# thisparticle/scl_slam

Measured on AMD Instinct MI355X. Metric: loop-closure candidates/sec: (scan, keyframe) pairs taken through full-database ARG-MIN detection per second (every pair aligned exactly and bounded by the f16 matrix-core screening; only the survivors get the f64 distance), batches of 16 scans, 10k-keyframe DB per GPU, higher is better.
Workload: dtype f64 results; f16-operand / f32-accumulate MFMA screening + f64 exact pass on the survivors

## Files before the change

### scl_slam_amd/csrc/engine.hip

```cpp
#include "scl_engine.h"

#include <hip/hip_runtime.h>

#include <cfloat>
#include <climits>
#include <chrono>
#include <cmath>
#include <cstdio>
#include <cstdlib>
#include <cstring>
#include <mutex>
#include <new>
#include <string>
#include <atomic>
#include <chrono>
#include <thread>
#include <vector>

#include "db_file.hpp"
#include "engine_internal.hpp"
#include "device_sort.hpp"
#include "plugin_host.hpp"

#ifdef SCL_DIAGNOSTICS
// ... 383 lines not shown
    return SCL_OK;
}

int topk_finish_locked(scl_engine *e, int k, bool have_dist, int *idx, float *d2, double *dist, int *shift, int *found)
{
    int rc;
    char *h = static_cast<char *>(e->h_pinned);
    bool seen = false;
    if (e->pinned_seq) {
        const volatile unsigned int *w = reinterpret_cast<const volatile unsigned int *>(h + cand_seq_offset(k));
        const auto t0 = std::chrono::steady_clock::now();
        int spins = 0;
        seen = true;
        while (*w != e->pinned_seq)
            if ((++spins & 255) == 0 && std::chrono::steady_clock::now() - t0 > std::chrono::microseconds(300)) { seen = false; break; }
        std::atomic_thread_fence(std::memory_order_acquire);
        if (seen) collect_profile(e);
    }
    if (!seen && (rc = sync_short(e))) return rc;
    const int *h_idx = reinterpret_cast<int *>(h);
    const float *h_d2 = reinterpret_cast<float *>(h + sizeof(int) * k);
    const double *h_dist = reinterpret_cast<double *>(h + (sizeof(int) + sizeof(float)) * k);
    const int *h_shift = reinterpret_cast<int *>(h + (sizeof(int) + sizeof(float) + sizeof(double)) * k);
    int nf = 0;
    for (int i = 0; i < k; ++i) {
        if (idx) idx[i] = h_idx[i];
        if (d2) d2[i] = h_d2[i];
        if (dist) dist[i] = have_dist ? h_dist[i] : kBigDist;
        if (shift) shift[i] = have_dist ? h_shift[i] : 0;
        if (h_idx[i] >= 0) nf++;
    }
    if (found) *found = nf;
    return SCL_OK;
}

int topk_with_distance_locked(scl_engine *e, int query, int lo, int hi, int k, float eps,
                              int *idx, float *d2, double *dist, int *shift, int *found)
{
    bool have_dist = false;
    int rc = topk_enqueue_locked(e, query, lo, hi, k, eps, dist || shift, &have_dist);
    if (rc) return rc;
    return topk_finish_locked(e, k, have_dist, idx, d2, dist, shift, found);
}

}

extern "C" {

const char *scl_status_string(int status)
{
    switch (status) {
    case SCL_OK: return "ok";
    case SCL_ERR_INVALID_ARG: return "invalid argument";
    case SCL_ERR_NO_DEVICE: return "no HIP device";
    case SCL_ERR_HIP: return "HIP runtime error";
    case SCL_ERR_OUT_OF_RANGE: return "index out of range";
    case SCL_ERR_NOMEM: return "out of memory";
    case SCL_ERR_UNSUPPORTED: return "unsupported";
    default: return "unknown status";
    }
}

const char *scl_last_error(const scl_engine *e) { return e ? e->last_error.c_str() : "null engine"; }

int scl_abi_version(void) { return 12; }

int scl_default_config(scl_config *c)
{
    if (!c) return SCL_ERR_INVALID_ARG;
    c->num_ring = 20; c->num_sector = 60; c->num_candidates = 3;
    c->dist_thres = 0.14; c->lidar_height = 1.65; c->max_radius = 80.0;
    c->num_exclude_recent = 100; c->tree_making_period = 10;
    c->search_ratio = 0.1;
    c->knn_exclude_eps = 0.0f;
    c->device = 0;
    c->initial_capacity = 4096;
    return SCL_OK;
}

static void log_env_overrides_once()
{
    static std::atomic<bool> done{false};
    if (done.exchange(true)) return;
    static const char *const names[] = {"SCL_SCREEN", "SCL_SCREEN_FORM", "SCL_SCREEN_V2_MIN", "SCL_SCREEN_PAIR", "SCL_RCCL_LIB",
                                        "SCL_SCREEN_VARIANT", "SCL_SCREEN_PROBE", "SCL_SCREEN_TAIL", "SCL_ALIGN_WGS",
                                        "SCL_ALIGN2_WGS", "SCL_ALIGN_FILTER", "SCL_SC_KERNEL", "SCL_SC_WAVES", "SCL_STAMP", "SCL_ABLATE",
                                        "SCL_ICP_REDUCE", "SCL_MATRIX_PLAIN", "SCL_MATRIX_KERNEL", "SCL_MATRIX_KR", "SCL_WIDE_EXACT", "SCL_STREAM_EXACT", "SCL_SMALL_EXACT_OFF",
                                        "SCL_SELF_ALIGN_OFF", "SCL_CAND_EXACT_OFF"};
    constexpr int kProduct = 5;
    int i = 0;
    for (const char *n : names) {
        const char *v = getenv(n);
#ifdef SCL_DIAGNOSTICS
        if (v) fprintf(stderr, "scl_engine (diagnostics build): environment override in effect: %s=%s\n", n, v);
#else
        if (v && i < kProduct) fprintf(stderr, "scl_engine: environment override in effect: %s=%s\n", n, v);
        else if (v) fprintf(stderr, "scl_engine: %s=%s is an experiment's switch: ignored by this build (make EXTRA=-DSCL_DIAGNOSTICS builds them in)\n", n, v);
#endif
        ++i;
    }
    (void)kProduct;
}

int scl_create(const scl_config *cfg, scl_engine **out)
{
    if (!cfg || !out) return SCL_ERR_INVALID_ARG;
    *out = nullptr;
    log_env_overrides_once();
    if (cfg->num_ring < 1 || cfg->num_ring > 256 || cfg->num_sector < 1 || cfg->num_sector > 1024 ||
        cfg->num_candidates < 1 || cfg->num_candidates > kTopkMaxK || cfg->tree_making_period < 1 ||
        cfg->num_exclude_recent < 0 || !(cfg->max_radius > 0.0) || !(cfg->search_ratio >= 0.0))
        return SCL_ERR_INVALID_ARG;
    int ndev = 0;
    if (hipGetDeviceCount(&ndev) != hipSuccess || ndev <= 0) return SCL_ERR_NO_DEVICE;
    if (cfg->device < 0 || cfg->device >= ndev) return SCL_ERR_INVALID_ARG;
    scl_engine *e = new (std::nothrow) scl_engine();
    if (!e) return SCL_ERR_NOMEM;
    e->cfg = *cfg;
    e->R = cfg->num_ring; e->S = cfg->num_sector;
    e->RG = (e->R + 3) / 4; e->R4 = e->RG * 4;
    e->hstride = hdesc_stride(e->RG, e->S);
    e->hkw = hkey_row_halfs(e->S);
    e->SR = (int)std::round(0.5 * cfg->search_ratio * (double)e->S);
    if (e->SR < 0) e->SR = 0;
    e->device = cfg->device;
    int rc = SCL_OK;
    auto bail = [&](int code) { scl_destroy(e); return code; };
    if (hipSetDevice(e->device) != hipSuccess) return bail(SCL_ERR_HIP);
    hipDeviceProp_t prop;
    if (hipGetDeviceProperties(&prop, e->device) == hipSuccess && prop.multiProcessorCount > 0)
        e->num_cu = prop.multiProcessorCount;
    if (hipStreamCreateWithFlags(&e->stream, hipStreamNonBlocking) != hipSuccess) return bail(SCL_ERR_HIP);
    {
        int lo_p = 0, hi_p = 0;
        (void)hipDeviceGetStreamPriorityRange(&lo_p, &hi_p);
        if (hipStreamCreateWithPriority(&e->stream2, hipStreamNonBlocking, hi_p) != hipSuccess) return bail(SCL_ERR_HIP);
    }
    if (hipEventCreateWithFlags(&e->ev_fork, hipEventDisableTiming) != hipSuccess) return bail(SCL_ERR_HIP);
    if (hipEventCreateWithFlags(&e->ev_join, hipEventDisableTiming) != hipSuccess) return bail(SCL_ERR_HIP);
    if (hipHostMalloc((void **)&e->h_out3, 64 * scl_engine::kSlots, hipHostMallocDefault) != hipSuccess) return bail(SCL_ERR_HIP);
    memset(e->h_out3, 0, 64 * scl_engine::kSlots);
    for (int i = 0; i < scl_engine::kSlots; ++i)
        if (hipEventCreateWithFlags(&e->ev_done[i], hipEventDisableTiming) != hipSuccess) return bail(SCL_ERR_HIP);
    if ((rc = ensure_capacity(e, 1))) return bail(rc);
    if ((rc = dev_alloc(e, &e->d_topk_scratch, (size_t)kTopkMaxBlocks * kTopkMaxK + 2))) return bail(rc);
    if (hipMemset(e->d_topk_scratch, 0, sizeof(unsigned long long) * ((size_t)kTopkMaxBlocks * kTopkMaxK + 2)) != hipSuccess) return bail(SCL_ERR_HIP);
    if ((rc = dev_alloc(e, &e->d_topk_idx, (size_t)kTopkMaxK * scl_engine::kScreenSets))) return bail(rc);
    if ((rc = dev_alloc(e, &e->d_topk_d2, (size_t)kTopkMaxK * scl_engine::kScreenSets))) return bail(rc);
    if ((rc = dev_alloc(e, &e->d_out3, (size_t)4))) return bail(rc);
    if ((rc = dev_alloc(e, &e->d_blk_part, (size_t)kTailBlocks * kTailRec * kMaxQueryBatch))) return bail(rc);
    static_assert(kMaxQueryBatch <= 4, "done_counter holds four counters");
    if ((rc = dev_alloc(e, &e->d_done_counter, (size_t)4))) return bail(rc);
    if (hipMemset(e->d_done_counter, 0, 16) != hipSuccess) return bail(SCL_ERR_HIP);
    {
        constexpr int NS = scl_engine::kScreenSets;
        if ((rc = dev_alloc(e, &e->d_nsurv, (size_t)NS))) return bail(rc);
        static_assert(NS <= kTminEpsOffset, "the launch's largest bound sits kTminEpsOffset words behind its t_min word");
        if ((rc = dev_alloc(e, &e->d_tmin, (size_t)NS + kTminEpsOffset))) return bail(rc);
        if (hipMemset(e->d_nsurv, 0, sizeof(int) * NS) != hipSuccess) return bail(SCL_ERR_HIP);
        if (hipMemset(e->d_tmin, 0xff, sizeof(unsigned int) * NS) != hipSuccess) return bail(SCL_ERR_HIP);
        if (hipMemset(e->d_tmin + NS, 0, sizeof(unsigned int) * kTminEpsOffset) != hipSuccess) return bail(SCL_ERR_HIP);
        if ((rc = dev_alloc(e, &e->d_surv_part, (size_t)NS * kSurvivorBlocks * kTailRec))) return bail(rc);
        if ((rc = dev_alloc(e, &e->d_surv_done, (size_t)NS))) return bail(rc);
        if (hipMemset(e->d_surv_done, 0, sizeof(unsigned int) * NS) != hipSuccess) return bail(SCL_ERR_HIP);
        if (hipMalloc(&e->d_surv_args, (size_t)8 * NS * kSurvivorArgBytes) != hipSuccess) return bail(SCL_ERR_NOMEM);
        if (hipHostMalloc(&e->h_surv_args, (size_t)8 * NS * kSurvivorArgBytes, hipHostMallocDefault) != hipSuccess) return bail(SCL_ERR_HIP);
        if (hipHostMalloc((void **)&e->h_stream_out, (size_t)2 * NS * 64, hipHostMallocDefault) != hipSuccess) return bail(SCL_ERR_HIP);
        for (auto &ev : e->ev_chunk) if (hipEventCreateWithFlags(&ev, hipEventDisableTiming) != hipSuccess) return bail(SCL_ERR_HIP);
        for (auto &ev : e->ev_k1) if (hipEventCreateWithFlags(&ev, hipEventDisableTiming) != hipSuccess) return bail(SCL_ERR_HIP);
        for (auto &ev : e->ev_sub0) if (hipEventCreateWithFlags(&ev, hipEventDisableTiming) != hipSuccess) return bail(SCL_ERR_HIP);
        if (hipEventCreateWithFlags(&e->ev_align_gate, hipEventDisableTiming) != hipSuccess) return bail(SCL_ERR_HIP);
        {
// ... 2470 lines not shown
```

### scl_slam_amd/csrc/sc_screen.hip

```cpp
#include <atomic>
#include <type_traits>

#include "align_exact.hpp"
#include "device_common.hpp"
#include "kernels.hpp"

namespace scl {

namespace {

typedef _Float16 h4 __attribute__((ext_vector_type(4)));
typedef _Float16 h8 __attribute__((ext_vector_type(8)));
typedef float f4v __attribute__((ext_vector_type(4)));
typedef float f2 __attribute__((ext_vector_type(2)));
typedef unsigned int u32x4 __attribute__((ext_vector_type(4)));
typedef u32x4 __attribute__((aligned(8))) u32x4_a8;

struct ScreenArgs {
    const double *vkey;
    const uint2 *hdesc; const unsigned int *kmask;
    const double *q_vkey; const float *q_rkey;
    const uint2 *q_hdesc; const unsigned int *q_kmask;
    const _Float16 *hkey; const _Float16 *q_hkey; int hkw;
    const float4 *rkey4; int rk_cap;
// ... 408 lines not shown
        const float v1 = hi[0], v2 = lo[0] + 7.0e-5f;
        int a1 = (int)(__float_as_uint(hi[0]) & 255u);
        const bool in_range = qnorm >= 1e-30f && qnorm <= 4.0e6f && knorm >= 1e-30f && knorm <= 4.0e6f &&
                              qnorm <= 1.0e4f * knorm && knorm <= 1.0e4f * qnorm;
        const float lead = (qerr > 0.f && kerr > 0.f) ? fminf(kAlign16Margin, 2.0f * (qerr + kerr + qerr * kerr) * 1.0001f + 1.6e-5f) : kAlign16Margin;
        bool uniq = use_filter && in_range && (v1 == v1) && (v2 < v1 - lead);
        const int ci = u_lo + idx - sq.base;
        const bool mine = q_live && ci >= 0 && ci < sq.n;
        unsigned long long amb = __builtin_amdgcn_ballot_w64(mine && !uniq) & 0xffffull;
        if (SCL_A2_PROBE != 1 && use_filter && amb) {
            const uint4 l0 = *reinterpret_cast<const uint4 *>(g_cur + 16 + IMG + loff0);
            uint4 l1 = make_uint4(0, 0, 0, 0);
            if (NLD > 1) l1 = *reinterpret_cast<const uint4 *>(g_cur + 16 + IMG + (ld1 ? loff1 : 0u));
            *reinterpret_cast<uint4 *>(smem_wave + IMG + loff0) = l0;
            if (ld1) *reinterpret_cast<uint4 *>(smem_wave + IMG + loff1) = l1;
            h8 bql[KS];
#pragma unroll
            for (int kk = 0; kk < KS; ++kk) bql[kk] = *reinterpret_cast<const h8 *>(qk + SK + 8 + 32 * kk + 8 * j4);
            wave_fence();
            float h2 = kNegInf, l2 = kNegInf;
            int g2 = 0;
#pragma unroll
            for (int t = 0; t < NT; ++t) {
                const int rho = t / NTAU, tau = t - rho * NTAU;
                const f4v zero = {0.f, 0.f, 0.f, 0.f};
                f4v hh = zero, xx = zero;
#pragma unroll
                for (int kk = 0; kk < KS; ++kk) {
                    const unsigned char *ap = smem_wave + rho * (CP * 2) + offs[kk + C::TSTEP * (NTAU - 1 - tau)];
                    const h8 ah = frag(ap), al = frag(ap + IMG);
                    const f4v one = __builtin_amdgcn_mfma_f32_16x16x32_f16(ah, bq[kk], zero, 0, 0, 0);
                    hh = kk == 0 ? one : hh + one;
                    xx = __builtin_amdgcn_mfma_f32_16x16x32_f16(ah, bql[kk], xx, 0, 0, 0);
                    xx = __builtin_amdgcn_mfma_f32_16x16x32_f16(al, bq[kk], xx, 0, 0, 0);
                }
#pragma unroll
                for (int i = 0; i < 4; ++i) {
                    const int sg = 16 * tau + 4 * j4 + i;
                    const float c = sg < C::ROWS ? __builtin_fmaf(xx[i], 0x1p-11f, hh[i]) : kNegInf;
                    l2 = fmaxf(l2, fminf(c, h2));
                    g2 = c > h2 ? P * sg + rho : g2;
                    h2 = fmaxf(h2, c);
                }
            }
#pragma unroll
            for (int off = 16; off <= 32; off <<= 1) {
                const float oh = __shfl_xor(h2, off, kWave), ol = __shfl_xor(l2, off, kWave);
                const int og = __shfl_xor(g2, off, kWave);
                l2 = fmaxf(fmaxf(l2, ol), fminf(h2, oh));
                g2 = oh > h2 ? og : g2;
                h2 = fmaxf(h2, oh);
            }
            if (!uniq && in_range && (h2 == h2) && (l2 < h2 - 2.0f * kAlignSplitEps)) { uniq = true; a1 = g2; }
            amb = __builtin_amdgcn_ballot_w64(mine && !uniq) & 0xffffull;
        }
        if (mine && j4 == 0 && uniq) starts_q[ci] = wrapS(a1 - SR, S);
        if (SCL_A2_PROBE == 1 && mine && j4 == 0 && !uniq) starts_q[ci] = kAlignUndecided;
        open_pairs += (unsigned long long)__popcll(amb);
        while (SCL_A2_PROBE != 1 && amb) {
            const int qn = __ffsll((long long)amb) - 1;
            amb &= amb - 1;
            const ScreenQuery oq = ab.q[qn];
            const double *vq = ab.vkey + (size_t)oq.slot * S;
            const double *vkp = ab.vkey + (size_t)(u_lo + idx) * S;
            double *vk2 = reinterpret_cast<double *>(smem_wave);
            int al;
            if constexpr (S / 2 <= kWave) {
                constexpr int L = S >> 1;
                const int ll = lane < L ? lane : L - 1;
                const double2 vk = *reinterpret_cast<const double2 *>(vkp + 2 * ll);
                al = align_keyframe_exact<S>(vk, lane, vk2, vq);
            } else {
                constexpr int SPL = (S + kWave - 1) / kWave, LA = S / SPL;
                const int ll = lane < LA ? lane : LA - 1;
                double vk[SPL];
#pragma unroll
                for (int u = 0; u < SPL; ++u) vk[u] = vkp[SPL * ll + u];
                al = align_keyframe_wide<S>(vk, lane, vk2, vq);
            }
            if (lane == 0) (ab.starts + (size_t)oq.buf * (size_t)ab.pair_stride)[u_lo + idx - oq.base] = wrapS(al - SR, S);
        }
    }
    if (lane == 0 && open_pairs && ab.fallbacks) atomicAdd(ab.fallbacks, open_pairs);
}

template <int RG, int S, int W>
__global__ __launch_bounds__(kScreenWaves * kWave, Align2Cfg<S>::OCC) void sc_align2_kernel(ScreenBatchArgs ab, const unsigned char *halign, int u_lo, int u_n)
{
    extern __shared__ __attribute__((aligned(16))) unsigned char smem_align2[];
    const int wave = __builtin_amdgcn_readfirstlane((int)(threadIdx.x >> 6));
    sc_align2_role<S, W>(ab, halign, u_lo, u_n, (int)blockIdx.x * kScreenWaves + wave, (int)gridDim.x * kScreenWaves,
                         smem_align2 + (size_t)wave * Align2Cfg<S>::LDS_WAVE);
}


template <int S>
__device__ __forceinline__ void rotate_mask(const unsigned long long (&m)[(S + 63) / 64], int s, unsigned long long (&out)[(S + 63) / 64])
{
    constexpr int NW = (S + 63) / 64;
    auto shr = [&](int k, unsigned long long (&o)[NW]) {
        const int w = k >> 6, b = k & 63;
#pragma unroll
        for (int i = 0; i < NW; ++i) {
            const unsigned long long lo = i + w < NW ? m[i + w] : 0ull, hi = i + w + 1 < NW ? m[i + w + 1] : 0ull;
            o[i] = b ? (lo >> b) | (hi << (64 - b)) : lo;
        }
    };
    auto shl = [&](int k, unsigned long long (&o)[NW]) {
        const int w = k >> 6, b = k & 63;
#pragma unroll
        for (int i = 0; i < NW; ++i) {
            const unsigned long long hi = i - w >= 0 && i - w < NW ? m[i - w] : 0ull, lo = i - w - 1 >= 0 && i - w - 1 < NW ? m[i - w - 1] : 0ull;
            o[i] = b ? (hi << b) | (lo >> (64 - b)) : hi;
        }
    };
    unsigned long long r1[NW], r2[NW];
    shr(s, r1);
    shl(S - s, r2);
#pragma unroll
    for (int i = 0; i < NW; ++i) {
        unsigned long long v = r1[i] | r2[i];
        const int top = S - 64 * i;
        if (top < 64) v &= top > 0 ? ((1ull << (top & 63)) - 1ull) : 0ull;
        out[i] = v;
    }
}

template <int RGH, int S, int W, int D, int PROBE>
__device__ __forceinline__ void sc_screen_role(const ScreenBatchArgs &ab, const int qi, const int bid, unsigned char *smem_raw)
{
    constexpr int NWV = kScreenWaves;
    constexpr int MT = (W + 15) / 16;
    constexpr int QSX = S + 16 * MT;
    constexpr int SB = RGH * 8;
    constexpr int KH = SB / 64;
    constexpr int QST = SB + 32;
    constexpr int HS = hdesc_stride_rgh(RGH, S);
    constexpr int SPW = S / NWV;
    constexpr int NST = SPW * KH;
    constexpr int NW64 = (S + 63) / 64;
    constexpr int MW = (NW64 + 1) / 2;
    static_assert(S % NWV == 0 && SB % 64 == 0 && NST % D == 0 && W <= 32 && S <= 224, "tiling");

    const int nbk = ab.nb;
    const ScreenArgs a = screen_args_of(ab, qi);
    const int lane = threadIdx.x & (kWave - 1);
    const int wave = __builtin_amdgcn_readfirstlane((int)(threadIdx.x >> 6));

    unsigned char *Qs = smem_raw;
    uint4 *rotq = reinterpret_cast<uint4 *>(Qs + (size_t)QSX * QST);
    unsigned char *tile = reinterpret_cast<unsigned char *>(rotq + S * MW) + (size_t)wave * (kGroup * kTileStride);
    f4v *part = reinterpret_cast<f4v *>(reinterpret_cast<unsigned char *>(rotq + S * MW) + (size_t)NWV * (kGroup * kTileStride));

    for (int idx = threadIdx.x; idx < QSX * (SB / 16); idx += blockDim.x) {
        const int cx = idx / (SB / 16), ch = idx - cx * (SB / 16);
        const int c = cx < S ? cx : cx - S;
        *reinterpret_cast<uint4 *>(Qs + (size_t)cx * QST + ch * 16) =
            *reinterpret_cast<const uint4 *>(reinterpret_cast<const unsigned char *>(a.q_hdesc) + (size_t)c * SB + ch * 16);
    }
    const bool q_bad = a.q_kmask[7] != 0;
    const float q_err = __uint_as_float(a.q_kmask[6]);
    {
        unsigned long long qm[NW64];
#pragma unroll
        for (int i = 0; i < NW64; ++i) qm[i] = (unsigned long long)a.q_kmask[2 * i] | ((unsigned long long)(2 * i + 1 < 7 ? a.q_kmask[2 * i + 1] : 0u) << 32);
        for (int sft = threadIdx.x; sft < S; sft += blockDim.x) {
// ... 833 lines not shown
template <int RG, int S, int W, bool MASKS = true, bool D2 = true>
__device__ __forceinline__ void sc_screen2_finish_body(const Screen2Args &fa, const int qi, const int chunk)
{
    constexpr int NW64 = (S + 63) / 64, MW = (NW64 + 1) / 2;
    const ScreenBatchArgs &ab = fa.prod;
    const ScreenArgs a = screen_args_of(ab, qi);
    __shared__ uint4 rotq[S * MW];
    __shared__ float wmin[4], wmax[4];
    __shared__ float4 qkey[D2 ? RG : 1];
    const int ci = (int)(chunk * blockDim.x + threadIdx.x);
    const bool live = ci < a.n;
    float4 qk_mine = make_float4(0.0f, 0.0f, 0.0f, 0.0f);
    if constexpr (D2) { if (threadIdx.x < RG) qk_mine = reinterpret_cast<const float4 *>(a.q_rkey)[threadIdx.x]; }
    FinishLoads<RG, S, W, D2> ld = sc_screen2_finish_request<RG, S, W, D2>(fa, a, qi, live ? ci : 0);
    build_rotq<S>(a.q_kmask, rotq, (int)threadIdx.x, (int)blockDim.x);
    const bool q_bad = a.q_kmask[7] != 0;
    if constexpr (D2) { if (threadIdx.x < RG) qkey[threadIdx.x] = qk_mine; }
    __syncthreads();
#pragma unroll
    for (int i = 0; i < FinishLoads<RG, S, W, D2>::NPF; ++i) asm("" : "+v"(ld.pv[i]));
    const float kInf = __int_as_float(0x7f800000);
    float contrib = kInf, peps = 0.0f;
    if (live) contrib = sc_screen2_finish_compute<RG, S, W, MASKS, D2>(a, ci, rotq, qkey, q_bad, __uint_as_float(a.q_kmask[6]), ld, peps);
    contrib = -wave_max_f32_dpp(-contrib);
    peps = wave_max_f32_dpp(peps);
    if ((threadIdx.x & 63) == 0) { wmin[threadIdx.x >> 6] = contrib; wmax[threadIdx.x >> 6] = peps; }
    __syncthreads();
    if (threadIdx.x == 0) {
        const float m = fminf(fminf(wmin[0], wmin[1]), fminf(wmin[2], wmin[3]));
        if (m < kInf) atomicMin(a.t_min, float_to_ordered_u(m));
        const float pe = fmaxf(fmaxf(wmax[0], wmax[1]), fmaxf(wmax[2], wmax[3]));
        if (pe > 0.0f) atomicMax(a.t_min + kTminEpsOffset, __float_as_uint(pe));
    }
}

__device__ __forceinline__ bool finish_block_of(const int fb, const int nq, const int chunks, int &qi, int &chunk)
{
    const int x = fb & 7, s = fb >> 3, g = s / nq;
    chunk = 8 * g + x; qi = s - g * nq;
    return chunk < chunks;
}
static int finish_blocks(int chunks, int nq) { return 8 * ((chunks + 7) / 8) * nq; }

template <int RG, int S, int W>
__global__ __launch_bounds__(256) void sc_screen2_finish_kernel(Screen2Args fa, int chunks)
{
    int qi, chunk;
    if (!finish_block_of((int)blockIdx.x, fa.prod.nq, chunks, qi, chunk)) return;
    sc_screen2_finish_body<RG, S, W>(fa, qi, chunk);
}

template <int RG, int S, int W>
__global__ __launch_bounds__(kScreenWaves * kWave, 2) void sc_screen2_tail_kernel(Screen2Args fa, ScreenBatchArgs nb, int align_blocks, int chunks)
{
    extern __shared__ __attribute__((aligned(16))) unsigned char smem_tail[];
    const int b = (int)blockIdx.x;
    if (b < align_blocks) { sc_align_role<RG, S, W>(nb, b, smem_tail); return; }
    int qi, chunk;
    if (!finish_block_of(b - align_blocks, fa.prod.nq, chunks, qi, chunk)) return;
    sc_screen2_finish_body<RG, S, W>(fa, qi, chunk);
}

template <int RG, int S, int W, bool MASKS = true, bool D2 = true>
__global__ __launch_bounds__(kScreenWaves * kWave, Align2Cfg<S>::OCC) void sc_screen2_tail2_kernel(Screen2Args fa, ScreenBatchArgs nb, const unsigned char *halign, int u_lo, int u_n,
                                                                                     int align_blocks, int chunks)
{
    extern __shared__ __attribute__((aligned(16))) unsigned char smem_tail2[];
#ifdef SCL_TAIL_FINISH_FIRST
    const int fblocks = (int)gridDim.x - align_blocks;
    const int b = (int)blockIdx.x < fblocks ? (int)blockIdx.x + align_blocks : (int)blockIdx.x - fblocks;
#else
    const int b = (int)blockIdx.x;
#endif
    if (b < align_blocks) {
        const int wave = __builtin_amdgcn_readfirstlane((int)(threadIdx.x >> 6));
        sc_align2_role<S, W>(nb, halign, u_lo, u_n, b * kScreenWaves + wave, align_blocks * kScreenWaves, smem_tail2 + (size_t)wave * Align2Cfg<S>::LDS_WAVE);
        return;
    }
    int qi, chunk;
    if (!finish_block_of(b - align_blocks, fa.prod.nq, chunks, qi, chunk)) return;
    sc_screen2_finish_body<RG, S, W, MASKS, D2>(fa, qi, chunk);
}

static bool screen_second_form()
{
    static const int form = [] { const char *e = getenv("SCL_SCREEN_FORM"); return e ? atoi(e) : 2; }();
    return form != 1;
}
static bool screen_pair_enabled()
{
    static const int on = [] { const char *e = getenv("SCL_SCREEN_PAIR"); return e ? atoi(e) : 1; }();
    return on != 0;
}
static int screen_v2_min_env()
{
    static const int v = [] { const char *e = getenv("SCL_SCREEN_V2_MIN"); return e ? atoi(e) : 0; }();
    return v;
}
int sc_screen_max_batch(const DbView &db, int SR)
{
    return (sc_screen_is_wide(db, SR) && screen_second_form()) ? S2Cfg<20, 180, 19>::NQ : kMaxScreenBatch;
}
size_t sc_screen_scratch_floats(const DbView &db, int SR)
{
    return sc_screen_is_wide(db, SR) ? (size_t)S2Cfg<20, 180, 19>::NQ * s2_part_floats<20, 180, 19>() : (size_t)S2Cfg<16, 120, 13>::NQ * s2_part_floats<16, 120, 13>();
}

static int fill_screen_args(const DbView &db, const ScreenBatch &sb, int align_filter, ScreenBatchArgs *ab)
{
    ab->vkey = db.vkey; ab->rkey = db.rkey; ab->hdesc = db.hdesc; ab->kmask = db.kmask; ab->rkey4 = db.rkey4; ab->hkey = db.hkey; ab->hkw = hkey_row_halfs(db.S);
    ab->starts = sb.starts; ab->approx = sb.approx; ab->ring_d2 = sb.ring_d2; ab->t_min = sb.t_min; ab->fallbacks = sb.align_fallbacks; ab->smask = sb.smask;
    ab->pair_stride = (unsigned long long)sb.pair_stride;
    ab->S = db.S; ab->R4 = 4 * db.RG; ab->hstride = db.hstride; ab->rk_cap = db.cap; ab->align_filter = align_filter;
    ab->nq = sb.nq;
    int nmax = 0;
    for (int i = 0; i < sb.nq; ++i) {
        if (sb.n[i] <= 0) return -1;
        ab->q[i] = ScreenQuery{sb.slot[i], sb.base[i], sb.n[i], sb.buf[i]};
        nmax = sb.n[i] > nmax ? sb.n[i] : nmax;
    }
    for (int i = sb.nq; i < kMaxScreenBatch; ++i) ab->q[i] = ab->q[0];
    return nmax;
}

struct ScreenPairMate { const ScreenBatch *sb; const ScreenBatch *next; };

template <int RG, int S, int W, int OCC0, int OCC1>
static hipError_t launch_screen_grid(const DbView &db, const ScreenBatch &sb, int align_filter, int num_cu, hipStream_t stream, int phases,
                                     const ScreenBatch *next, const ScreenPairMate *mate = nullptr)
{
    constexpr int RGH = hdesc_rgh(RG);
    ScreenBatchArgs ab{};
    const int nmax = fill_screen_args(db, sb, align_filter, &ab);
    if (nmax < 0) return hipErrorInvalidValue;
    ScreenBatchArgs ab_m{};
    const int nmax_m = mate ? fill_screen_args(db, *mate->sb, align_filter, &ab_m) : 0;
    if (nmax_m < 0) return hipErrorInvalidValue;
    const int ngroups = (nmax + kGroup - 1) / kGroup;
    static_assert(halign_bytes(S) > 0, "alignment image");
    if (db.hstride != hdesc_stride(RG, S) || !sb.starts || !db.halign) return hipErrorInvalidValue;
    static std::atomic<bool> attr_set_dev[64];
    int dev_ = 0; (void)hipGetDevice(&dev_);
    std::atomic<bool> &attr_set = attr_set_dev[dev_ & 63];
    static const int variant = scl_lab_int("SCL_SCREEN_VARIANT", 0);
    void (*kern)(ScreenFusedArgs) = sc_screen_kernel<RG, S, W, 15, OCC0>;
#ifdef SCL_DIAGNOSTICS
    if (variant == 1) kern = sc_screen_kernel<RG, S, W, 15, OCC1>;
    if (variant == 2) kern = sc_screen_kernel<RG, S, W, 5, OCC0>;
    static const int probe = scl_lab_int("SCL_SCREEN_PROBE", 0);
    if (probe == 2) kern = sc_screen_kernel<RG, S, W, 15, OCC0, 2>;
#else
    const int probe = 0;
#endif
    constexpr int MTA = (S + 15) / 16, MT = (W + 15) / 16, QSX = S + 16 * MT, MW = ((S + 63) / 64 + 1) / 2;
    const size_t lds0 = (size_t)S * 8 + (size_t)(32 * MTA) * 4 + (size_t)2 * (16 * MTA + hkey_halfs(S) + 8) * 2 +
                        (size_t)kScreenWaves * ((2 * S + 2) * 8);
    const size_t lds1 = (size_t)QSX * (RGH * 8 + 32) + (size_t)S * MW * 16 + (size_t)kScreenWaves * kGroup * kTileStride +
                        (size_t)(2 * kScreenWaves * MT) * kWave * 16;
    if (!attr_set.load(std::memory_order_acquire)) {
        hipError_t e = hipFuncSetAttribute((const void *)sc_screen_kernel<RG, S, W, 15, OCC0>, hipFuncAttributeMaxDynamicSharedMemorySize, 128 * 1024);
        if (e == hipSuccess) e = hipFuncSetAttribute((const void *)sc_align_kernel<RG, S, W>, hipFuncAttributeMaxDynamicSharedMemorySize, 128 * 1024);
        if (e != hipSuccess) return e;
#ifdef SCL_DIAGNOSTICS
        (void)hipFuncSetAttribute((const void *)sc_screen_kernel<RG, S, W, 15, OCC1>, hipFuncAttributeMaxDynamicSharedMemorySize, 128 * 1024);
        (void)hipFuncSetAttribute((const void *)sc_screen_kernel<RG, S, W, 5, OCC0>, hipFuncAttributeMaxDynamicSharedMemorySize, 128 * 1024);
        (void)hipFuncSetAttribute((const void *)sc_screen_kernel<RG, S, W, 15, OCC0, 2>, hipFuncAttributeMaxDynamicSharedMemorySize, 128 * 1024);
#endif
        attr_set.store(true, std::memory_order_release);
    }
    auto align_blocks = [&](int groups, int nq, bool beside_products) {
        int b = (groups + kScreenWaves - 1) / kScreenWaves;
        static const int cap_env = scl_lab_int("SCL_ALIGN_WGS", 0);
        int cap = cap_env > 0 ? cap_env : (beside_products ? 2 * num_cu / (nq > 0 ? nq : 1) : num_cu);
        if (cap < 1) cap = 1;
        return b > cap ? cap : b;
// ... 36 lines not shown
        hipError_t e = hipGetLastError();
        if (e != hipSuccess) return e;
    }
    if (probe == 4 || !(phases & kScreenProducts)) return hipSuccess;
    if (use_v2) {
        static std::atomic<bool> attr2_dev[64];
        std::atomic<bool> &attr2 = attr2_dev[dev_ & 63];
        if (!attr2.load(std::memory_order_acquire)) {
            hipError_t e = hipFuncSetAttribute((const void *)sc_screen2_kernel<RG, S, W>, hipFuncAttributeMaxDynamicSharedMemorySize, (int)(s2_lds<RG, S, W>()));
            if (e != hipSuccess) return e;
            attr2.store(true, std::memory_order_release);
        }
        Screen2Args f2{}, f2_m{};
        f2.prod = ab; f2.part = sb.part;
        union_of(sb, &f2.u_lo, &f2.u_n);
        const int WGU = 8 * S2Cfg<RG, S, W>::NP * (mate ? 2 : 1);
        int nwg = (num_cu / WGU) * WGU;
        if (nwg < WGU) nwg = WGU;
        f2.nwg = nwg;
        hipError_t e = hipSuccess;
        if constexpr (kPairGrid) {
            if (mate) {
                static std::atomic<bool> attrp_dev[64];
                std::atomic<bool> &attrp = attrp_dev[dev_ & 63];
                if (!attrp.load(std::memory_order_acquire)) {
                    e = hipFuncSetAttribute((const void *)sc_screen2_kernel<RG, S, W, 2>, hipFuncAttributeMaxDynamicSharedMemorySize, (int)(s2_lds<RG, S, W>()));
                    if (e != hipSuccess) return e;
                    attrp.store(true, std::memory_order_release);
                }
                f2_m.prod = ab_m; f2_m.part = mate->sb->part; f2_m.nwg = nwg;
                union_of(*mate->sb, &f2_m.u_lo, &f2_m.u_n);
                Screen2PairArgs fp{};
                fp.prod[0] = ab; fp.prod[1] = ab_m; fp.part[0] = sb.part; fp.part[1] = mate->sb->part; fp.nwg = nwg;
                const int hi0 = f2.u_lo + f2.u_n, hi1 = f2_m.u_lo + f2_m.u_n;
                fp.u_lo = f2.u_lo < f2_m.u_lo ? f2.u_lo : f2_m.u_lo;
                fp.u_n = (hi0 > hi1 ? hi0 : hi1) - fp.u_lo;
                hipLaunchKernelGGL((sc_screen2_kernel<RG, S, W, 2>), dim3(nwg), dim3(S2Cfg<RG, S, W>::WV * kWave), (s2_lds<RG, S, W>()), stream, fp);
            }
        }
        if (!mate) hipLaunchKernelGGL((sc_screen2_kernel<RG, S, W>), dim3(nwg), dim3(S2Cfg<RG, S, W>::WV * kWave), (s2_lds<RG, S, W>()), stream, f2);
        if ((e = hipGetLastError()) != hipSuccess) return e;
        auto launch_tail = [&](const ScreenBatch &sb, const Screen2Args &f2, const int nmax, const ScreenBatch *next) -> hipError_t {
            const bool next_v2 = next && second_form_for(*next);
            const int chunks = (nmax + 255) / 256;
            const dim3 fgrid(finish_blocks(chunks, sb.nq)), ablock(kScreenWaves * kWave);
            if (!next) {
                hipLaunchKernelGGL((sc_screen2_finish_kernel<RG, S, W>), fgrid, dim3(256), 0, stream, f2, chunks);
                return hipGetLastError();
            }
            if (next->nq < 1 || next->nq > kMaxScreenBatch) return hipErrorInvalidValue;
            ScreenBatchArgs nb{};
            const int nmax2 = fill_screen_args(db, *next, align_filter, &nb);
            if (nmax2 < 0) return hipErrorInvalidValue;
            nb.skip_d2 = next_v2 ? 1 : 0;
            int ulo = 0, un = 0, ablocks;
            if (next_v2) {
                union_of(*next, &ulo, &un);
                ablocks = align2_blocks(un);
            } else {
                const int ng2 = (nmax2 + kGroup - 1) / kGroup;
                int per_q = 3 * num_cu / next->nq;
                per_q = per_q < 1 ? 1 : per_q;
                nb.nb = (ng2 + kScreenWaves - 1) / kScreenWaves;
                nb.nb = nb.nb > per_q ? per_q : nb.nb;
                ablocks = nb.nb * next->nq;
            }
            static const int tail_env = scl_lab_int("SCL_SCREEN_TAIL", 1);
            if (tail_env) {
                const dim3 tgrid(ablocks + finish_blocks(chunks, sb.nq));
                const bool d2 = !sb.no_ring_metric;
                if (!next_v2) hipLaunchKernelGGL((sc_screen2_tail_kernel<RG, S, W>), tgrid, ablock, lds0, stream, f2, nb, ablocks, chunks);
                else if (sb.smask && d2) hipLaunchKernelGGL((sc_screen2_tail2_kernel<RG, S, W, true, true>), tgrid, ablock, lds_a2, stream, f2, nb, db.halign, ulo, un, ablocks, chunks);
                else if (sb.smask) hipLaunchKernelGGL((sc_screen2_tail2_kernel<RG, S, W, true, false>), tgrid, ablock, lds_a2, stream, f2, nb, db.halign, ulo, un, ablocks, chunks);
                else if (d2) hipLaunchKernelGGL((sc_screen2_tail2_kernel<RG, S, W, false, true>), tgrid, ablock, lds_a2, stream, f2, nb, db.halign, ulo, un, ablocks, chunks);
                else hipLaunchKernelGGL((sc_screen2_tail2_kernel<RG, S, W, false, false>), tgrid, ablock, lds_a2, stream, f2, nb, db.halign, ulo, un, ablocks, chunks);
                return hipGetLastError();
            }
            hipLaunchKernelGGL((sc_screen2_finish_kernel<RG, S, W>), fgrid, dim3(256), 0, stream, f2, chunks);
            if ((e = hipGetLastError()) != hipSuccess) return e;
            if (next_v2) hipLaunchKernelGGL((sc_align2_kernel<RG, S, W>), dim3(ablocks), ablock, lds_a2, stream, nb, db.halign, ulo, un);
            else hipLaunchKernelGGL((sc_align_kernel<RG, S, W>), dim3(ablocks), ablock, lds0, stream, nb);
            return hipGetLastError();
        };
        if ((e = launch_tail(sb, f2, nmax, next)) != hipSuccess || !mate) return e;
        return launch_tail(*mate->sb, f2_m, nmax_m, mate->next);
    }
    ScreenFusedArgs fa{};
    fa.prod = ab;
    int blocks = num_cu * 2;
    if (blocks > ngroups) blocks = ngroups;
    if (blocks > kScreenMaxBlocks) blocks = kScreenMaxBlocks;
    fa.prod.nb = blocks;
    fa.prod.self_align = self_align ? 1 : 0;
    int extra = 0;
    if (next && probe != 3) {
        if (next->nq < 1 || next->nq > kMaxScreenBatch) return hipErrorInvalidValue;
        const int nmax2 = fill_screen_args(db, *next, align_filter, &fa.next);
        if (nmax2 < 0) return hipErrorInvalidValue;
        fa.next.skip_d2 = next_v2 ? 1 : 0;
        fa.next.nb = align_blocks((nmax2 + kGroup - 1) / kGroup, next->nq, true);
        extra = fa.next.nb * next->nq;
#ifdef SCL_DIAGNOSTICS
        if (probe == 5 || probe == 6) fa.next.align_filter = probe == 5 ? 2 : 3;
#endif
    }
    const size_t lds = (extra || self_align) && lds0 > lds1 ? lds0 : lds1;
    fa.align_blocks = extra;
    const int patterned = fused_patterned_blocks(sb.nq, blocks, extra);
    const int slots = 8 * ((blocks + 7) >> 3);
    const int grid = patterned + (extra > slots ? extra - slots : 0);
    hipLaunchKernelGGL(kern, dim3(grid), dim3(kScreenWaves * kWave), lds, stream, fa);
    return hipGetLastError();
}

hipError_t launch_sc_screen_batch(const DbView &db, const ScreenBatch &sb, int SR, int align_filter, int num_cu, hipStream_t stream, int phases,
                                  const ScreenBatch *next)
{
    if (sb.nq < 1 || sb.nq > kMaxScreenBatch || !sc_screen_supported(db, SR)) return hipErrorInvalidValue;
    if (sc_screen_is_wide(db, SR)) return launch_screen_grid<20, 180, 19, 2, 2>(db, sb, align_filter, num_cu, stream, phases, next);
    return launch_screen_grid<16, 120, 13, 2, 3>(db, sb, align_filter, num_cu, stream, phases, next);
}

bool sc_screen_pairs(const DbView &db, int SR)
{
    return sc_screen_supported(db, SR) && !sc_screen_is_wide(db, SR) && screen_second_form() && screen_pair_enabled() && screen_v2_min_env() <= kMaxScreenBatch &&
           scl_lab_int("SCL_SCREEN_VARIANT", 0) == 0 && scl_lab_int("SCL_SCREEN_PROBE", 0) == 0;
}

hipError_t launch_sc_screen_pair(const DbView &db, const ScreenBatch &sb0, const ScreenBatch &sb1, int SR, int align_filter, int num_cu, hipStream_t stream,
                                 const ScreenBatch *next0, const ScreenBatch *next1)
{
    if (!sc_screen_pairs(db, SR) || sb0.nq != kMaxScreenBatch || sb1.nq != kMaxScreenBatch) return hipErrorInvalidValue;
    const ScreenPairMate mate{&sb1, next1};
    return launch_screen_grid<16, 120, 13, 2, 3>(db, sb0, align_filter, num_cu, stream, kScreenProducts, next0, &mate);
}

}

#ifdef S2_STAMP
extern "C" int scl_debug_s2_stamps(unsigned long long *out)
{
    return (int)hipMemcpyFromSymbol(out, HIP_SYMBOL(scl::g_s2_stamps), sizeof(unsigned long long) * 4 * 64);
}
#endif
```

Baseline: 2.711 billion.

## Fuse paired-batch screen tails into one kernel sharing keyframe alignment images

When two batches are screened as a pair, their two tail launches (finish plus next-batch f16 alignment) are merged into a single kernel. The alignment role loads each keyframe's alignment image into LDS once and runs the MFMA shift search against both batches' queries over the union of their keyframe ranges. This removes one kernel launch and halves the image loads and LDS staging for the alignment stage. The cost is more registers for two query sets and a larger union range, which may include keyframes that only one batch needs.

After: 2.971 billion, median of 6. 9.6% higher.

```diff
diff --git a/scl_slam_amd/csrc/engine.hip b/scl_slam_amd/csrc/engine.hip
--- a/scl_slam_amd/csrc/engine.hip
+++ b/scl_slam_amd/csrc/engine.hip
@@ -489,12 +489,12 @@
 {
     static std::atomic<bool> done{false};
     if (done.exchange(true)) return;
-    static const char *const names[] = {"SCL_SCREEN", "SCL_SCREEN_FORM", "SCL_SCREEN_V2_MIN", "SCL_SCREEN_PAIR", "SCL_RCCL_LIB",
+    static const char *const names[] = {"SCL_SCREEN", "SCL_SCREEN_FORM", "SCL_SCREEN_V2_MIN", "SCL_SCREEN_PAIR", "SCL_TAIL_PAIR", "SCL_RCCL_LIB",
                                         "SCL_SCREEN_VARIANT", "SCL_SCREEN_PROBE", "SCL_SCREEN_TAIL", "SCL_ALIGN_WGS",
                                         "SCL_ALIGN2_WGS", "SCL_ALIGN_FILTER", "SCL_SC_KERNEL", "SCL_SC_WAVES", "SCL_STAMP", "SCL_ABLATE",
                                         "SCL_ICP_REDUCE", "SCL_MATRIX_PLAIN", "SCL_MATRIX_KERNEL", "SCL_MATRIX_KR", "SCL_WIDE_EXACT", "SCL_STREAM_EXACT", "SCL_SMALL_EXACT_OFF",
                                         "SCL_SELF_ALIGN_OFF", "SCL_CAND_EXACT_OFF"};
-    constexpr int kProduct = 5;
+    constexpr int kProduct = 6;
     int i = 0;
     for (const char *n : names) {
         const char *v = getenv(n);
diff --git a/scl_slam_amd/csrc/sc_screen.hip b/scl_slam_amd/csrc/sc_screen.hip
--- a/scl_slam_amd/csrc/sc_screen.hip
+++ b/scl_slam_amd/csrc/sc_screen.hip
@@ -514,6 +514,232 @@
         }
     }
     if (lane == 0 && open_pairs && ab.fallbacks) atomicAdd(ab.fallbacks, open_pairs);
+}
+
+template <int S, int W>
+__device__ __forceinline__ void sc_align2_pair_role(const ScreenBatchArgs *abs, const unsigned char *halign, int u_lo, int u_n,
+                                                    const int wave_global, const int waves_total, unsigned char *smem_wave)
+{
+    using C = Align2Cfg<S>;
+    constexpr int P = C::P, CP = C::CP, KS = C::KS, NTAU = C::NTAU, NT = C::NT, ND = C::ND, IMG = C::IMG, SK = C::SK, NLD = C::NLD;
+    static_assert(P == 4 || P == 8, "alignment image");
+    static_assert(S % P == 0 && (16 * P) % 32 == 0 && CP >= S + 8 && IMG % 16 == 0 && S <= 256 && NLD >= 1 && NLD <= 2, "tiling of the shifts");
+    constexpr int NS = 2;
+    constexpr int SR = (W - 1) / 2;
+    constexpr int HAB = halign_bytes(S);
+    const int lane = threadIdx.x & (kWave - 1);
+    const int c16 = lane & 15, j4 = lane >> 4;
+    int q_base[NS], q_n[NS], q_buf[NS];
+    h8 bq[NS][KS];
+    float qnorm[NS], qerr[NS];
+#pragma unroll
+    for (int s = 0; s < NS; ++s) {
+        const ScreenBatchArgs &ab = abs[s];
+        const int cq = c16 < ab.nq ? c16 : 0;
+        const ScreenQuery sq = ab.q[cq];
+        q_base[s] = sq.base; q_n[s] = c16 < ab.nq ? sq.n : 0;
+        q_buf[s] = sq.buf;
+        const _Float16 *qk = reinterpret_cast<const _Float16 *>(ab.hkey) + (size_t)sq.slot * (size_t)ab.hkw;
+#pragma unroll
+        for (int kk = 0; kk < KS; ++kk) bq[s][kk] = *reinterpret_cast<const h8 *>(qk + 32 * kk + 8 * j4);
+        qnorm[s] = *reinterpret_cast<const float *>(qk + SK);
+        qerr[s] = *reinterpret_cast<const float *>(qk + SK + 2);
+    }
+    unsigned int offs[ND];
+    {
+        int base0 = (8 * j4 - P * c16) % S; base0 = base0 < 0 ? base0 + S : base0;
+#pragma unroll
+        for (int d = 0; d < ND; ++d) {
+            int x = (base0 + 32 * (d - C::TSTEP * (NTAU - 1))) % S; x = x < 0 ? x + S : x;
+            offs[d] = (unsigned int)(2 * x);
+        }
+    }
+    const bool use_filter = abs[0].align_filter != 0;
+    const float kNegInf = __int_as_float(0xff800000);
+    unsigned long long open_pairs[NS];
+#pragma unroll
+    for (int s = 0; s < NS; ++s) open_pairs[s] = 0;
+    auto frag = [&](const unsigned char *ap) -> h8 {
+        if constexpr (P == 8) return *reinterpret_cast<const h8 *>(ap);
+        else {
+            const uint2 a0 = *reinterpret_cast<const uint2 *>(ap), a1 = *reinterpret_cast<const uint2 *>(ap + 8);
+            const u32x4 aw = {a0.x, a0.y, a1.x, a1.y};
+            return __builtin_bit_cast(h8, aw);
+        }
+    };
+    const unsigned int loff0 = (unsigned int)lane * 16u, loff1 = (unsigned int)(kWave + lane) * 16u;
+    const bool ld1 = NLD > 1 && loff1 < (unsigned int)IMG;
+    uint4 pre0 = make_uint4(0, 0, 0, 0), pre1 = make_uint4(0, 0, 0, 0);
+    float knorm_pre = 0.f, kerr_pre = 0.f;
+    auto image_of = [&](int idx) { idx = idx < u_n ? idx : u_n - 1; return halign + (size_t)(u_lo + idx) * (size_t)HAB; };
+    if (wave_global < u_n) {
+        const unsigned char *g = image_of(wave_global);
+        pre0 = *reinterpret_cast<const uint4 *>(g + 16 + loff0);
+        if (NLD > 1) pre1 = *reinterpret_cast<const uint4 *>(g + 16 + (ld1 ? loff1 : 0u));
+        knorm_pre = *reinterpret_cast<const float *>(g);
+        kerr_pre = *reinterpret_cast<const float *>(g + 4);
+    }
+    for (int idx = wave_global; idx < u_n; idx += waves_total) {
+        wave_fence();
+        *reinterpret_cast<uint4 *>(smem_wave + loff0) = pre0;
+        if (ld1) *reinterpret_cast<uint4 *>(smem_wave + loff1) = pre1;
+        const float knorm = knorm_pre, kerr = kerr_pre;
+        wave_fence();
+        const unsigned char *g_cur = image_of(idx);
+        {
+            const unsigned char *g = image_of(idx + waves_total);
+            pre0 = *reinterpret_cast<const uint4 *>(g + 16 + loff0);
+            if (NLD > 1) pre1 = *reinterpret_cast<const uint4 *>(g + 16 + (ld1 ? loff1 : 0u));
+            knorm_pre = *reinterpret_cast<const float *>(g);
+            kerr_pre = *reinterpret_cast<const float *>(g + 4);
+        }
+        float hi[NS][2], lo[NS][2];
+#pragma unroll
+        for (int s = 0; s < NS; ++s) { hi[s][0] = hi[s][1] = kNegInf; lo[s][0] = lo[s][1] = kNegInf; }
+        h8 af[2][KS];
+#pragma unroll
+        for (int kk = 0; kk < KS; ++kk) af[0][kk] = frag(smem_wave + offs[kk + C::TSTEP * (NTAU - 1)]);
+#pragma unroll
+        for (int t = 0; t < NT; ++t) {
+            const int rho = t / NTAU, tau = t - rho * NTAU;
+            if (t + 1 < NT) {
+                const int rn = (t + 1) / NTAU, tn = (t + 1) - rn * NTAU;
+#pragma unroll
+                for (int kk = 0; kk < KS; ++kk) af[(t + 1) & 1][kk] = frag(smem_wave + rn * (CP * 2) + offs[kk + C::TSTEP * (NTAU - 1 - tn)]);
+            }
+            const int ch = t & 1;
+#pragma unroll
+            for (int s = 0; s < NS; ++s) {
+                f4v acc = {0.f, 0.f, 0.f, 0.f};
+#pragma unroll
+                for (int kk = 0; kk < KS; ++kk) acc = __builtin_amdgcn_mfma_f32_16x16x32_f16(af[t & 1][kk], bq[s][kk], acc, 0, 0, 0);
+#pragma unroll
+                for (int i = 0; i < 4; i += 2) {
+                    const int sg0 = 16 * tau + 4 * j4 + i, sg1 = sg0 + 1;
+                    const float x = sg0 < C::ROWS ? __uint_as_float((__float_as_uint(acc[i]) & ~255u) | (unsigned int)(P * sg0 + rho)) : kNegInf;
+                    const float y = sg1 < C::ROWS ? __uint_as_float((__float_as_uint(acc[i + 1]) & ~255u) | (unsigned int)(P * sg1 + rho)) : kNegInf;
+                    lo[s][ch] = fmaxf(lo[s][ch], __builtin_amdgcn_fmed3f(hi[s][ch], x, y));
+                    hi[s][ch] = fmaxf(fmaxf(hi[s][ch], x), y);
+                }
+            }
+        }
+        auto merge = [](float &h, float &l, float oh, float ol) { l = fmaxf(fmaxf(l, ol), fminf(h, oh)); h = fmaxf(h, oh); };
+        bool in_range[NS], uniq[NS], mine[NS];
+        int a1[NS];
+        unsigned long long amb[NS];
+        bool any_open = false;
+#pragma unroll
+        for (int s = 0; s < NS; ++s) {
+            merge(hi[s][0], lo[s][0], hi[s][1], lo[s][1]);
+#pragma unroll
+            for (int off = 16; off <= 32; off <<= 1) merge(hi[s][0], lo[s][0], __shfl_xor(hi[s][0], off, kWave), __shfl_xor(lo[s][0], off, kWave));
+            const float v1 = hi[s][0], v2 = lo[s][0] + 7.0e-5f;
+            a1[s] = (int)(__float_as_uint(hi[s][0]) & 255u);
+            in_range[s] = qnorm[s] >= 1e-30f && qnorm[s] <= 4.0e6f && knorm >= 1e-30f && knorm <= 4.0e6f &&
+                          qnorm[s] <= 1.0e4f * knorm && knorm <= 1.0e4f * qnorm[s];
+            const float lead = (qerr[s] > 0.f && kerr > 0.f) ? fminf(kAlign16Margin, 2.0f * (qerr[s] + kerr + qerr[s] * kerr) * 1.0001f + 1.6e-5f) : kAlign16Margin;
+            uniq[s] = use_filter && in_range[s] && (v1 == v1) && (v2 < v1 - lead);
+            const int ci = u_lo + idx - q_base[s];
+            mine[s] = ci >= 0 && ci < q_n[s];
+            amb[s] = __builtin_amdgcn_ballot_w64(mine[s] && !uniq[s]) & 0xffffull;
+            any_open = any_open || amb[s] != 0;
+        }
+        if (SCL_A2_PROBE != 1 && use_filter && any_open) {
+            int ln = (int)(threadIdx.x & (kWave - 1));
+            asm volatile("" : "+v"(ln));
+            const unsigned int lo0 = (unsigned int)ln * 16u, lo1 = (unsigned int)(kWave + ln) * 16u;
+            const bool l1_in = NLD > 1 && lo1 < (unsigned int)IMG;
+            const uint4 l0 = *reinterpret_cast<const uint4 *>(g_cur + 16 + IMG + lo0);
+            uint4 l1 = make_uint4(0, 0, 0, 0);
+            if (NLD > 1) l1 = *reinterpret_cast<const uint4 *>(g_cur + 16 + IMG + (l1_in ? lo1 : 0u));
+            *reinterpret_cast<uint4 *>(smem_wave + IMG + lo0) = l0;
+            if (l1_in) *reinterpret_cast<uint4 *>(smem_wave + IMG + lo1) = l1;
+            const int c16o = ln & 15, j4o = ln >> 4;
+#pragma unroll
+            for (int s = 0; s < NS; ++s) {
+                if (!amb[s]) continue;
+                const _Float16 *qk = reinterpret_cast<const _Float16 *>(abs[s].hkey) + (size_t)abs[s].q[c16o < abs[s].nq ? c16o : 0].slot * (size_t)abs[s].hkw;
+                h8 bql[KS];
+#pragma unroll
+                for (int kk = 0; kk < KS; ++kk) bql[kk] = *reinterpret_cast<const h8 *>(qk + SK + 8 + 32 * kk + 8 * j4o);
+                wave_fence();
+                float h2 = kNegInf, l2 = kNegInf;
+                int g2 = 0;
+#pragma unroll
+                for (int t = 0; t < NT; ++t) {
+                    const int rho = t / NTAU, tau = t - rho * NTAU;
+                    const f4v zero = {0.f, 0.f, 0.f, 0.f};
+                    f4v hh = zero, xx = zero;
+#pragma unroll
+                    for (int kk = 0; kk < KS; ++kk) {
+                        const unsigned char *ap = smem_wave + rho * (CP * 2) + offs[kk + C::TSTEP * (NTAU - 1 - tau)];
+                        const h8 ah = frag(ap), al = frag(ap + IMG);
+                        const f4v one = __builtin_amdgcn_mfma_f32_16x16x32_f16(ah, bq[s][kk], zero, 0, 0, 0);
+                        hh = kk == 0 ? one : hh + one;
+                        xx = __builtin_amdgcn_mfma_f32_16x16x32_f16(ah, bql[kk], xx, 0, 0, 0);
+                        xx = __builtin_amdgcn_mfma_f32_16x16x32_f16(al, bq[s][kk], xx, 0, 0, 0);
+                    }
+#pragma unroll
+                    for (int i = 0; i < 4; ++i) {
+                        const int sg = 16 * tau + 4 * j4 + i;
+                        const float c = sg < C::ROWS ? __builtin_fmaf(xx[i], 0x1p-11f, hh[i]) : kNegInf;
+                        l2 = fmaxf(l2, fminf(c, h2));
+                        g2 = c > h2 ? P * sg + rho : g2;
+                        h2 = fmaxf(h2, c);
+                    }
+                }
+#pragma unroll
+                for (int off = 16; off <= 32; off <<= 1) {
+                    const float oh = __shfl_xor(h2, off, kWave), ol = __shfl_xor(l2, off, kWave);
+                    const int og = __shfl_xor(g2, off, kWave);
+                    l2 = fmaxf(fmaxf(l2, ol), fminf(h2, oh));
+                    g2 = oh > h2 ? og : g2;
+                    h2 = fmaxf(h2, oh);
+                }
+                if (!uniq[s] && in_range[s] && (h2 == h2) && (l2 < h2 - 2.0f * kAlignSplitEps)) { uniq[s] = true; a1[s] = g2; }
+                amb[s] = __builtin_amdgcn_ballot_w64(mine[s] && !uniq[s]) & 0xffffull;
+            }
+        }
+#pragma unroll
+        for (int s = 0; s < NS; ++s) {
+            const ScreenBatchArgs &ab = abs[s];
+            const int ci = u_lo + idx - q_base[s];
+            int buf = q_buf[s];
+            asm volatile("" : "+v"(buf));
+            int *starts_q = ab.starts + (size_t)buf * (size_t)ab.pair_stride;
+            if (mine[s] && j4 == 0 && uniq[s]) starts_q[ci] = wrapS(a1[s] - SR, S);
+            if (SCL_A2_PROBE == 1 && mine[s] && j4 == 0 && !uniq[s]) starts_q[ci] = kAlignUndecided;
+            open_pairs[s] += (unsigned long long)__popcll(amb[s]);
+            while (SCL_A2_PROBE != 1 && amb[s]) {
+                const int qn = __ffsll((long long)amb[s]) - 1;
+                amb[s] &= amb[s] - 1;
+                int lane = (int)(threadIdx.x & (kWave - 1));
+                asm volatile("" : "+v"(lane));
+                const ScreenQuery oq = ab.q[qn];
+                const double *vq = ab.vkey + (size_t)oq.slot * S;
+                const double *vkp = ab.vkey + (size_t)(u_lo + idx) * S;
+                double *vk2 = reinterpret_cast<double *>(smem_wave);
+                int al;
+                if constexpr (S / 2 <= kWave) {
+                    constexpr int L = S >> 1;
+                    const int ll = lane < L ? lane : L - 1;
+                    const double2 vk = *reinterpret_cast<const double2 *>(vkp + 2 * ll);
+                    al = align_keyframe_exact<S>(vk, lane, vk2, vq);
+                } else {
+                    constexpr int SPL = (S + kWave - 1) / kWave, LA = S / SPL;
+                    const int ll = lane < LA ? lane : LA - 1;
+                    double vk[SPL];
+#pragma unroll
+                    for (int u = 0; u < SPL; ++u) vk[u] = vkp[SPL * ll + u];
+                    al = align_keyframe_wide<S>(vk, lane, vk2, vq);
+                }
+                if (lane == 0) (ab.starts + (size_t)oq.buf * (size_t)ab.pair_stride)[u_lo + idx - oq.base] = wrapS(al - SR, S);
+            }
+        }
+    }
+#pragma unroll
+    for (int s = 0; s < NS; ++s)
+        if ((threadIdx.x & (kWave - 1)) == 0 && open_pairs[s] && abs[s].fallbacks) atomicAdd(abs[s].fallbacks, open_pairs[s]);
 }
 
 template <int RG, int S, int W>
@@ -1513,6 +1739,43 @@
     sc_screen2_finish_body<RG, S, W, MASKS, D2>(fa, qi, chunk);
 }
 
+struct TailPairArgs {
+    Screen2Args fin[2];
+    ScreenBatchArgs nb[2];
+    const unsigned char *halign;
+    int u_lo, u_n;
+    int align_blocks, align_sets;
+    int chunks[2], chunks_max;
+};
+static_assert(sizeof(TailPairArgs) <= 2048, "a kernel's arguments end at 4 KB");
+
+template <int RG, int S, int W, bool MASKS, bool D2>
+__global__ __launch_bounds__(kScreenWaves * kWave, 3) void sc_screen2_tail_pair_kernel(TailPairArgs ta)
+{
+    extern __shared__ __attribute__((aligned(16))) unsigned char smem_tailp[];
+    const int b = (int)blockIdx.x;
+    if (b < ta.align_blocks) {
+        const int wave = __builtin_amdgcn_readfirstlane((int)(threadIdx.x >> 6));
+        unsigned char *tile = smem_tailp + (size_t)wave * Align2Cfg<S>::LDS_WAVE;
+        const int wg = b * kScreenWaves + wave, wt = ta.align_blocks * kScreenWaves;
+        if (ta.align_sets == 2) sc_align2_pair_role<S, W>(ta.nb, ta.halign, ta.u_lo, ta.u_n, wg, wt, tile);
+#ifdef SCL_DIAGNOSTICS
+        else if (ta.align_sets == -2) {
+            sc_align2_role<S, W>(ta.nb[0], ta.halign, ta.u_lo, ta.u_n, wg, wt, tile);
+            sc_align2_role<S, W>(ta.nb[1], ta.halign, ta.u_lo, ta.u_n, wg, wt, tile);
+        }
+#endif
+        else sc_align2_role<S, W>(ta.nb[0], ta.halign, ta.u_lo, ta.u_n, wg, wt, tile);
+        return;
+    }
+    int qi, chunk;
+    const int nq0 = ta.fin[0].prod.nq;
+    if (!finish_block_of(b - ta.align_blocks, nq0 + ta.fin[1].prod.nq, ta.chunks_max, qi, chunk)) return;
+    const int set = qi < nq0 ? 0 : 1;
+    if (chunk >= ta.chunks[set]) return;
+    sc_screen2_finish_body<RG, S, W, MASKS, D2>(ta.fin[set], qi - (set ? nq0 : 0), chunk);
+}
+
 static bool screen_second_form()
 {
     static const int form = [] { const char *e = getenv("SCL_SCREEN_FORM"); return e ? atoi(e) : 2; }();
@@ -1522,6 +1785,11 @@
 {
     static const int on = [] { const char *e = getenv("SCL_SCREEN_PAIR"); return e ? atoi(e) : 1; }();
     return on != 0;
+}
+static int screen_tail_pair()
+{
+    static const int v = [] { const char *e = getenv("SCL_TAIL_PAIR"); return e ? atoi(e) : 1; }();
+    return v;
 }
 static int screen_v2_min_env()
 {
@@ -1724,6 +1992,35 @@
             else hipLaunchKernelGGL((sc_align_kernel<RG, S, W>), dim3(ablocks), ablock, lds0, stream, nb);
             return hipGetLastError();
         };
+        if constexpr (kPairGrid) {
+            const int tp = screen_tail_pair();
+            const ScreenBatch *n0 = next, *n1 = mate ? mate->next : nullptr;
+            if (mate && tp != 0 && n0 && second_form_for(*n0) && (!n1 || second_form_for(*n1)) &&
+                !sb.smask && !mate->sb->smask && !sb.no_ring_metric && !mate->sb->no_ring_metric) {
+                TailPairArgs ta{};
+                ta.fin[0] = f2; ta.fin[1] = f2_m; ta.halign = db.halign;
+                int lo = 0, hi = 0;
+                const ScreenBatch *nx[2] = {n0, n1};
+                for (int s = 0; s < (n1 ? 2 : 1); ++s) {
+                    if (fill_screen_args(db, *nx[s], align_filter, &ta.nb[s]) < 0) return hipErrorInvalidValue;
+                    ta.nb[s].skip_d2 = 1;
+                    int ulo, un;
+                    union_of(*nx[s], &ulo, &un);
+                    if (s == 0) { lo = ulo; hi = ulo + un; } else { lo = ulo < lo ? ulo : lo; hi = ulo + un > hi ? ulo + un : hi; }
+                }
+                ta.u_lo = lo; ta.u_n = hi - lo;
+                ta.align_sets = n1 ? 2 : 1;
+#ifdef SCL_DIAGNOSTICS
+                if (n1 && tp == 2) ta.align_sets = -2;
+#endif
+                ta.align_blocks = align2_blocks(ta.u_n);
+                ta.chunks[0] = (nmax + 255) / 256; ta.chunks[1] = (nmax_m + 255) / 256;
+                ta.chunks_max = ta.chunks[0] > ta.chunks[1] ? ta.chunks[0] : ta.chunks[1];
+                const dim3 tgrid(ta.align_blocks + finish_blocks(ta.chunks_max, sb.nq + mate->sb->nq));
+                hipLaunchKernelGGL((sc_screen2_tail_pair_kernel<RG, S, W, false, true>), tgrid, dim3(kScreenWaves * kWave), lds_a2, stream, ta);
+                return hipGetLastError();
+            }
+        }
         if ((e = launch_tail(sb, f2, nmax, next)) != hipSuccess || !mate) return e;
         return launch_tail(*mate->sb, f2_m, nmax_m, mate->next);
     }
```
